# zyddnys/sd_animation_optical_flow

Hardware: AMD Instinct MI355X
Metric: frame-pairs/sec (flow+warp+mask) at 512x768 (higher is better)
Workload: dtype f32

## Files before the change

sd_animation_optical_flow_amd/csrc/conv_wino.hip:

```cpp
#include "ofx_internal.h"

#include <cmath>
#include <cstdlib>
#include <cstring>

namespace {

constexpr int kWBK = 16;
constexpr int kLDV = kWBK + 4;
constexpr int kOOB = 0x7FFFFFF0;

template <int W_, int H_, int LDH, int Y0, int X0> struct Halo {
    static constexpr int W = W_, H = H_, ldh = LDH, y_org = Y0, x_org = X0;
    static constexpr int pix = W * H;
    static constexpr int items = pix * (kWBK / 4);
    static constexpr int slots = (items + 255) / 256;
    static constexpr int floats = pix * ldh;
};
using Halo3x3 = Halo<18, 10, 24, -1, -1>;
template <bool VERT> using Halo15 = Halo<VERT ? 16 : 20, VERT ? 12 : 8, VERT ? 16 : 20, VERT ? -2 : 0, VERT ? 0 : -2>;

struct WinoK {
    const float* in0;
    const float* in1;
    const float* u;
    const float* scale;
    const float* shift;
    const float* addend;
    const float* res;
    const float* nmean;
    const float* nrstd;
    float* stats;
    float* out;
    float* aux_z;
    float* aux_rh;
    float* aux_h;
    int ld0, c0, ld1, cin, ldo, ldadd, ldh, ldres;
    int H, W, Cout, act;
    int nblk;
    int nb32;
    int tpr, tpi, mtiles;
    int bytes0, bytes1, bytesu;
    float alpha;
};

struct Patch {
    int nb, pb, y0, x0;
};

__device__ __forceinline__ Patch wino_patch(const WinoK& p) {
    const int nblk = p.mtiles * p.nblk;
    const int bid = blockIdx.x;
    const int q8 = nblk >> 3, r8 = nblk & 7;
    const int xcd = bid & 7, idx = bid >> 3;
    const int L = (xcd < r8 ? xcd * (q8 + 1) : r8 * (q8 + 1) + (xcd - r8) * q8) + idx;
    const int nb = L % p.nblk, mt = L / p.nblk;
    const int pb = mt / p.tpi;
    const int trem = mt - pb * p.tpi;
    const int py = trem / p.tpr;
    return {nb, pb, py * 8, (trem - py * p.tpr) * 16};
}

template <class ALG, bool NORM = false>
__device__ __forceinline__ void wino_slabs(const WinoK& p, const Patch& pt, float* Hs, float* Vs, int tid, int wave,
                                           f32x16 (&acc)[ALG::P][ALG::NT]) {
    typedef int v4i __attribute__((ext_vector_type(4)));
    using HALO = typename ALG::HALO;
    constexpr int P = ALG::P, NT = ALG::NT;
    const int lane = tid & 63;

    const float* in1s = p.in1 ? p.in1 : p.in0;
    const int bytes1s = p.in1 ? p.bytes1 : p.bytes0;
    int hpix[HALO::slots];
    unsigned hok = 0;
#pragma unroll
    for (int k = 0; k < HALO::slots; ++k) {
        const int i = tid + 256 * k;
        const int pix = i >> 2;
        const int hy = pix / HALO::W, hx = pix - hy * HALO::W;
        const int gy = pt.y0 + HALO::y_org + hy, gx = pt.x0 + HALO::x_org + hx;
        const bool ok = i < HALO::items && (unsigned)gy < (unsigned)p.H && (unsigned)gx < (unsigned)p.W;
        hpix[k] = ok ? (pt.pb * p.H + gy) * p.W + gx : 0;
        hok |= (ok ? 1u : 0u) << k;
    }
    const int hq = (tid & 3) * 16;
    float4 pa[HALO::slots];
    float4 pmu, prs;
    auto a_issue = [&](int cb) __attribute__((always_inline)) {
        const int c = cb * kWBK;
        const bool s0 = c < p.c0;
        const __amdgpu_buffer_rsrc_t rs = __builtin_amdgcn_make_buffer_rsrc((void*)(s0 ? p.in0 : in1s), (short)0, s0 ? p.bytes0 : bytes1s, 0x00020000);
        const int so = (s0 ? c : c - p.c0) * 4;
        const int ldb = (s0 ? p.ld0 : p.ld1) * 4;
#pragma unroll
        for (int k = 0; k < HALO::slots; ++k) {
            const int vo = ((hok >> k) & 1u) ? hpix[k] * ldb + hq : kOOB;
            v4i t = __builtin_amdgcn_raw_buffer_load_b128(rs, vo, so, 0);
            pa[k] = *reinterpret_cast<float4*>(&t);
        }
        if constexpr (NORM) {
            const long at = (long)pt.pb * p.c0 + c + (tid & 3) * 4;
            pmu = *reinterpret_cast<const float4*>(p.nmean + at);
            prs = *reinterpret_cast<const float4*>(p.nrstd + at);
        }
    };

    const __amdgpu_buffer_rsrc_t rsu = __builtin_amdgcn_make_buffer_rsrc((void*)p.u, (short)0, p.bytesu, 0x00020000);
    const int c8n = p.cin >> 3;
    const int wlane = lane * 16;
    const int pt0 = ALG::pt0(wave), blk0 = ALG::blk0(pt.nb, wave);
    float4 wr[P][NT][2];
    auto w_issue = [&](int q, int cb) __attribute__((always_inline)) {
#pragma unroll
        for (int nt = 0; nt < NT; ++nt)
#pragma unroll
            for (int ks = 0; ks < 2; ++ks) {
                const int so = (((pt0 + q) * p.nb32 + blk0 + nt) * c8n + 2 * cb + ks) * 1024;
                v4i t = __builtin_amdgcn_raw_buffer_load_b128(rsu, wlane, so, 0);
                wr[q][nt][ks] = *reinterpret_cast<float4*>(&t);
            }
    };

#pragma unroll
    for (int q = 0; q < P; ++q)
#pragma unroll
        for (int nt = 0; nt < NT; ++nt)
#pragma unroll
            for (int e = 0; e < 16; ++e) acc[q][nt][e] = 0.f;

    const ALG xf(Hs, Vs, tid, wave);
    const float* const afrag = Vs + (pt0 * 32 + (lane & 31)) * kLDV + 4 * (lane >> 5);

    const int CB = p.cin / kWBK;
    a_issue(0);
#pragma unroll
    for (int q = 0; q < P; ++q) w_issue(q, 0);
    for (int cb = 0; cb < CB; ++cb) {
        const int nx = cb + 1 < CB ? cb + 1 : cb;
#pragma unroll
        for (int k = 0; k < HALO::slots; ++k) {
            const int i = tid + 256 * k;
            if (HALO::slots * 256 > HALO::items && k == HALO::slots - 1 && i >= HALO::items) break;
            float4 v = pa[k];
            if constexpr (NORM) {
                v.x = fmaxf((v.x - pmu.x) * prs.x, 0.f);
                v.y = fmaxf((v.y - pmu.y) * prs.y, 0.f);
                v.z = fmaxf((v.z - pmu.z) * prs.z, 0.f);
                v.w = fmaxf((v.w - pmu.w) * prs.w, 0.f);
                if (!((hok >> k) & 1u)) v = make_float4(0.f, 0.f, 0.f, 0.f);
            }
            *reinterpret_cast<float4*>(&Hs[(i >> 2) * HALO::ldh + (i & 3) * 4]) = v;
        }
        __syncthreads();
        xf();
        __syncthreads();
        a_issue(nx);
        __builtin_amdgcn_sched_barrier(0);
#pragma unroll
        for (int q = 0; q < P; ++q) {
#pragma unroll
            for (int ks = 0; ks < 2; ++ks) {
                const float4 a = *reinterpret_cast<const float4*>(afrag + q * 32 * kLDV + 8 * ks);
#pragma unroll
                for (int nt = 0; nt < NT; ++nt) {
                    const float4 b = wr[q][nt][ks];
                    acc[q][nt] = __builtin_amdgcn_mfma_f32_32x32x2f32(a.x, b.x, acc[q][nt], 0, 0, 0);
                    acc[q][nt] = __builtin_amdgcn_mfma_f32_32x32x2f32(a.y, b.y, acc[q][nt], 0, 0, 0);
                    acc[q][nt] = __builtin_amdgcn_mfma_f32_32x32x2f32(a.z, b.z, acc[q][nt], 0, 0, 0);
                    acc[q][nt] = __builtin_amdgcn_mfma_f32_32x32x2f32(a.w, b.w, acc[q][nt], 0, 0, 0);
                }
            }
            w_issue(q, nx);
        }
    }
}

__device__ __forceinline__ float2 f2(float a, float b) { return make_float2(a, b); }
__device__ __forceinline__ float2 operator+(float2 a, float2 b) { return f2(a.x + b.x, a.y + b.y); }
__device__ __forceinline__ float2 operator-(float2 a, float2 b) { return f2(a.x - b.x, a.y - b.y); }
__device__ __forceinline__ float2 operator*(float s, float2 a) { return f2(s * a.x, s * a.y); }

struct Wino3x3 {
    using HALO = Halo3x3;
    static constexpr int P = 4, NT = 2;
    __device__ static int pt0(int wave) { return 4 * wave; }
    __device__ static int blk0(int nb, int) { return 2 * nb; }
    const float* src;
    float* dst;
    __device__ __forceinline__ Wino3x3(const float* Hs, float* Vs, int tid, int wave) {
        const int ttx = (tid & 63) >> 3, tcp = tid & 7;
        src = Hs + (2 * wave * HALO::W + 2 * ttx) * HALO::ldh + 2 * tcp;
        dst = Vs + (wave * 8 + ttx) * kLDV + 2 * tcp;
    }
    __device__ __forceinline__ void operator()() const {
        float2 d[4][4];
#pragma unroll
        for (int r = 0; r < 4; ++r)
#pragma unroll
            for (int c = 0; c < 4; ++c) d[r][c] = *reinterpret_cast<const float2*>(src + (r * HALO::W + c) * HALO::ldh);
        float2 t[4][4];
#pragma unroll
        for (int c = 0; c < 4; ++c) {
            t[0][c] = d[0][c] - d[2][c];
            t[1][c] = d[1][c] + d[2][c];
            t[2][c] = d[2][c] - d[1][c];
            t[3][c] = d[1][c] - d[3][c];
        }
#pragma unroll
        for (int i = 0; i < 4; ++i) {
            float2 v[4];
            v[0] = t[i][0] - t[i][2];
            v[1] = t[i][1] + t[i][2];
            v[2] = t[i][2] - t[i][1];
            v[3] = t[i][1] - t[i][3];
#pragma unroll
            for (int j = 0; j < 4; ++j) *reinterpret_cast<float2*>(dst + (i * 4 + j) * 32 * kLDV) = v[j];
        }
    }
};

template <bool VERT> struct Wino15 {
    using HALO = Halo15<VERT>;
    static constexpr int P = 8, NT = 1;
    __device__ static int pt0(int) { return 0; }
    __device__ static int blk0(int nb, int wave) { return 4 * nb + wave; }
    static constexpr int tap = (VERT ? HALO::W : 1) * HALO::ldh;
    const float* src;
    float* dst;
    __device__ static int base(int t) { return VERT ? (4 * (t >> 4)) * HALO::W + (t & 15) : (t >> 2) * HALO::W + 4 * (t & 3); }
    __device__ static int oy(int t, int i) { return VERT ? 4 * (t >> 4) + i : t >> 2; }
    __device__ static int ox(int t, int i) { return VERT ? (t & 15) : 4 * (t & 3) + i; }
    __device__ __forceinline__ Wino15(const float* Hs, float* Vs, int tid, int) {
        const int ttile = tid >> 3, tcp = tid & 7;
        src = Hs + base(ttile) * HALO::ldh + 2 * tcp;
        dst = Vs + ttile * kLDV + 2 * tcp;
    }
    __device__ __forceinline__ void operator()() const {
        float2 d[8];
#pragma unroll
        for (int j = 0; j < 8; ++j) d[j] = *reinterpret_cast<const float2*>(src + j * tap);
        float2 v[8];
        v[0] = (d[0] - d[6]) + 5.25f * (d[4] - d[2]);
        v[7] = (d[7] - d[1]) + 5.25f * (d[3] - d[5]);
        float2 te = (d[2] + d[6]) - 4.25f * d[4], to = (d[1] + d[5]) - 4.25f * d[3];
        v[1] = te + to;
        v[2] = te - to;
        te = (0.25f * d[2] + d[6]) - 1.25f * d[4];
        to = (0.5f * d[1] - 2.5f * d[3]) + 2.0f * d[5];
        v[3] = te + to;
        v[4] = te - to;
        te = (4.0f * d[2] + d[6]) - 5.0f * d[4];
        to = (2.0f * d[1] - 2.5f * d[3]) + 0.5f * d[5];
        v[5] = te + to;
        v[6] = te - to;
#pragma unroll
        for (int j = 0; j < 8; ++j) *reinterpret_cast<float2*>(dst + j * 32 * kLDV) = v[j];
    }
};

constexpr int kLDX = 32;
constexpr int kVF2 = 16 * 32 * kLDV;
constexpr int kSmem2 = Halo3x3::floats + kVF2;
constexpr int kXF = 4 * 2 * 32 * kLDX;
static_assert(kXF + 2 * 4 * 32 * 2 <= kSmem2, "exchange and statistics must fit");

template <bool NORM, bool RES, bool STATS>
__global__ __launch_bounds__(256, 2) void wino_conv_kernel(const WinoK p) {
    __shared__ __attribute__((aligned(16))) float smem[kSmem2];
    float* const Hs = smem;
    float* const Vs = smem + Halo3x3::floats;
    const int tid = threadIdx.x, lane = tid & 63;
    const int wave = __builtin_amdgcn_readfirstlane(tid >> 6);
    const Patch pt = wino_patch(p);
    f32x16 acc[4][2];
    wino_slabs<Wino3x3, NORM>(p, pt, Hs, Vs, tid, wave, acc);

    const float act_lo = p.act == OFX_ACT_RELU ? 0.0f : -3.402823466e38f;
    float* const X = smem;
    float* const Sx = smem + kXF;
    const int on = tid & 31, otx = tid >> 5;
#pragma unroll
    for (int nt = 0; nt < 2; ++nt) {
        __syncthreads();
#pragma unroll
        for (int e = 0; e < 16; ++e) {
            const int tile = (e & 3) + 8 * (e >> 2) + 4 * (lane >> 5);
            const float m0 = acc[0][nt][e], m1 = acc[1][nt][e], m2 = acc[2][nt][e], m3 = acc[3][nt][e];
            X[((wave * 2 + 0) * 32 + tile) * kLDX + (lane & 31)] = m0 + m1 + m2;
            X[((wave * 2 + 1) * 32 + tile) * kLDX + (lane & 31)] = m1 - m2 - m3;
        }
        __syncthreads();
        const int oc = pt.nb * 64 + nt * 32 + on;
        if (oc < p.Cout) {
            const float sc = (p.scale ? p.scale[oc] : 1.0f) * p.alpha;
            const float sh = p.shift ? p.shift[oc] : 0.0f;
            float st_s = 0.0f, st_q = 0.0f;
#pragma unroll
            for (int ty = 0; ty < 4; ++ty) {
                const int tile = ty * 8 + otx;
                float x[4][2];
#pragma unroll
                for (int w = 0; w < 4; ++w)
#pragma unroll
                    for (int j = 0; j < 2; ++j) x[w][j] = X[((w * 2 + j) * 32 + tile) * kLDX + on];
                float r[2][2];
                if constexpr (RES) {
#pragma unroll
                    for (int a = 0; a < 2; ++a)
#pragma unroll
                        for (int j = 0; j < 2; ++j)
                            r[a][j] = p.res[(((long)pt.pb * p.H + pt.y0 + 2 * ty + a) * p.W + pt.x0 + 2 * otx + j) * p.ldres + oc];
                }
#pragma unroll
                for (int a = 0; a < 2; ++a)
#pragma unroll
                    for (int j = 0; j < 2; ++j) {
                        const float y = a == 0 ? x[0][j] + x[1][j] + x[2][j] : x[1][j] - x[2][j] - x[3][j];
                        const long pix = ((long)pt.pb * p.H + pt.y0 + 2 * ty + a) * p.W + pt.x0 + 2 * otx + j;
                        float v = fmaxf(y * sc + sh, act_lo);
                        if constexpr (RES) v = fmaxf(v + r[a][j], 0.0f);
                        p.out[pix * p.ldo + oc] = v;
                        if constexpr (STATS) {
                            st_s += v;
                            st_q = fmaf(v, v, st_q);
                        }
                    }
            }
            if constexpr (STATS) {
                st_s += __shfl_xor(st_s, 32, 64);
                st_q += __shfl_xor(st_q, 32, 64);
                if (lane < 32) {
                    Sx[((nt * 4 + wave) * 32 + on) * 2 + 0] = st_s;
                    Sx[((nt * 4 + wave) * 32 + on) * 2 + 1] = st_q;
                }
            }
        }
    }
    if constexpr (STATS) {
        __syncthreads();
        const int nt = tid >> 5;
        const int oc = pt.nb * 64 + nt * 32 + on;
        if (tid < 64 && oc < p.Cout) {
            float s = 0.0f, q = 0.0f;
#pragma unroll
            for (int w = 0; w < 4; ++w) {
                s += Sx[((nt * 4 + w) * 32 + on) * 2 + 0];
                q += Sx[((nt * 4 + w) * 32 + on) * 2 + 1];
            }
            const long row = (long)pt.pb * p.tpi + (pt.y0 >> 3) * p.tpr + (pt.x0 >> 4);
            p.stats[(row * p.Cout + oc) * 2 + 0] = s;
            p.stats[(row * p.Cout + oc) * 2 + 1] = q;
        }
    }
}

int launch3x3(const WinoK& k, dim3 grid, dim3 block, hipStream_t s) {
    const int v = (k.nmean ? 4 : 0) | (k.res ? 2 : 0) | (k.stats ? 1 : 0);
    switch (v) {
        case 0: OFX_LAUNCH((wino_conv_kernel<false, false, false>), grid, block, s, k); break;
        case 1: OFX_LAUNCH((wino_conv_kernel<false, false, true>), grid, block, s, k); break;
        case 2: OFX_LAUNCH((wino_conv_kernel<false, true, false>), grid, block, s, k); break;
        case 4: OFX_LAUNCH((wino_conv_kernel<true, false, false>), grid, block, s, k); break;
        case 5: OFX_LAUNCH((wino_conv_kernel<true, false, true>), grid, block, s, k); break;
        case 6: OFX_LAUNCH((wino_conv_kernel<true, true, false>), grid, block, s, k); break;
        default: return OFX_EINVAL;
    }
    return ofx_launch_status();
}

template <bool VERT, int EPI>
__global__ __launch_bounds__(256, 2) void wino15_conv_kernel(const WinoK p) {
    using T = Wino15<VERT>;
    using HALO = typename T::HALO;
    __shared__ __attribute__((aligned(16))) float smem[HALO::floats + 8 * 32 * kLDV];
    float* const Hs = smem;
    float* const Vs = smem + HALO::floats;
    const int tid = threadIdx.x, lane = tid & 63;
    const int wave = __builtin_amdgcn_readfirstlane(tid >> 6);
    const Patch pt = wino_patch(p);
    f32x16 acc[8][1];
    wino_slabs<T>(p, pt, Hs, Vs, tid, wave, acc);

    const int n = pt.nb * 128 + wave * 32 + (lane & 31);
    if (n >= p.Cout) return;
    const float sc = (p.scale ? p.scale[n] : 1.0f) * p.alpha;
    const float sh = p.shift ? p.shift[n] : 0.0f;
    const float act_lo = p.act == OFX_ACT_RELU ? 0.0f : -3.402823466e38f;
    const int hd = p.Cout >> 1;
    const bool r_half = EPI == OFX_EPI_GRU_ZR && pt.nb * 128 >= hd;
#pragma unroll
    for (int eb = 0; eb < 16; eb += 4) {
        long pix[4][4];
        float y[4][4], ad[4][4], x1[4][4], x2[4][4];
#pragma unroll
        for (int u = 0; u < 4; ++u) {
            const int e = eb + u;
            const int tile = (e & 3) + 8 * (e >> 2) + 4 * (lane >> 5);
#pragma unroll
            for (int i = 0; i < 4; ++i) pix[u][i] = ((long)pt.pb * p.H + pt.y0 + T::oy(tile, i)) * p.W + pt.x0 + T::ox(tile, i);
            const float m0 = acc[0][0][e], m1 = acc[1][0][e], m2 = acc[2][0][e], m3 = acc[3][0][e];
            const float m4 = acc[4][0][e], m5 = acc[5][0][e], m6 = acc[6][0][e], m7 = acc[7][0][e];
            const float s12 = m1 + m2, d12 = m1 - m2, s34 = m3 + m4, d34 = m3 - m4, s56 = m5 + m6, d56 = m5 - m6;
            y[u][0] = m0 + s12 + s34 + s56;
            y[u][1] = d12 + 2.0f * d34 + 0.5f * d56;
            y[u][2] = s12 + 4.0f * s34 + 0.25f * s56;
            y[u][3] = d12 + 8.0f * d34 + 0.125f * d56 + m7;
        }
#pragma unroll
        for (int u = 0; u < 4; ++u)
#pragma unroll
            for (int i = 0; i < 4; ++i) {
                ad[u][i] = p.addend ? p.addend[pix[u][i] * p.ldadd + n] : 0.0f;
                x1[u][i] = EPI == OFX_EPI_GRU_ZR ? (r_half ? p.aux_h[pix[u][i] * p.ldh + n - hd] : 1.0f)
                           : EPI == OFX_EPI_GRU_Q ? p.aux_z[pix[u][i] * p.Cout + n] : 0.0f;
                x2[u][i] = EPI == OFX_EPI_GRU_Q ? p.aux_h[pix[u][i] * p.ldh + n] : 0.0f;
            }
#pragma unroll
        for (int u = 0; u < 4; ++u)
#pragma unroll
            for (int i = 0; i < 4; ++i) {
                const float v = y[u][i] * sc + sh + ad[u][i];
                if (EPI == OFX_EPI_PLAIN) {
                    p.out[pix[u][i] * p.ldo + n] = fmaxf(v, act_lo);
                } else if (EPI == OFX_EPI_GRU_ZR) {
                    const float g = ofx_sigmoid(v) * x1[u][i];
                    if (r_half) p.aux_rh[pix[u][i] * hd + n - hd] = g;
                    else p.aux_z[pix[u][i] * hd + n] = g;
                } else {
                    p.aux_h[pix[u][i] * p.ldh + n] = (1.0f - x1[u][i]) * x2[u][i] + x1[u][i] * ofx_tanh(v);
                }
            }
    }
}

template <bool VERT>
int launch15(const WinoK& k, int epi, dim3 grid, dim3 block, hipStream_t s) {
    switch (epi) {
        case OFX_EPI_PLAIN: OFX_LAUNCH((wino15_conv_kernel<VERT, OFX_EPI_PLAIN>), grid, block, s, k); break;
        case OFX_EPI_GRU_ZR: OFX_LAUNCH((wino15_conv_kernel<VERT, OFX_EPI_GRU_ZR>), grid, block, s, k); break;
        case OFX_EPI_GRU_Q: OFX_LAUNCH((wino15_conv_kernel<VERT, OFX_EPI_GRU_Q>), grid, block, s, k); break;
        default: return OFX_EINVAL;
    }
    return ofx_launch_status();
}

bool is_3x3(const ofx_conv_desc* d) { return d->KH == 3 && d->KW == 3; }
bool is_1d(int KH, int KW) { return (KH == 1 && KW == 5) || (KH == 5 && KW == 1); }
int wino_points(const ofx_conv_desc* d) { return is_3x3(d) ? 16 : 8; }
int wino_cblk(const ofx_conv_desc* d) { return is_3x3(d) ? 64 : 128; }

}

bool ofx_conv_wino_fits(const ofx_conv_desc* d) {
    const int cin = d->c0 + d->c1;
    const bool plain = d->epi == OFX_EPI_PLAIN && d->out != nullptr && d->ldo >= d->Cout && (d->act == OFX_ACT_NONE || d->act == OFX_ACT_RELU);
    bool shape_epi = false;
    if (is_3x3(d)) {
        shape_epi = d->padH == 1 && d->padW == 1 && plain && !d->addend && (!d->res || d->ldres >= d->Cout) &&
                    (!d->nmean || (d->nrstd && !d->in1 && ofx_aligned16(d->nmean) && ofx_aligned16(d->nrstd)));
    } else if (is_1d(d->KH, d->KW)) {
        shape_epi = d->padH == d->KH / 2 && d->padW == d->KW / 2 && !d->nmean && !d->res &&
                    (plain || (d->epi == OFX_EPI_GRU_ZR && (d->Cout / 2) % 128 == 0) || d->epi == OFX_EPI_GRU_Q);
    }
    return shape_epi && d->precision == OFX_PREC_FP32 && (d->nz <= 1) && d->stride == 1 && d->Hout == d->Hin && d->Wout == d->Win &&
           d->Hin % 8 == 0 && d->Win % 16 == 0 && cin % kWBK == 0 && d->c0 % kWBK == 0 &&
           d->wino_w != nullptr && ofx_aligned16(d->wino_w);
}

int ofx_conv_wino_stats_rows(const ofx_conv_desc* d) {
    return is_3x3(d) && d->act == OFX_ACT_NONE && !d->res ? (d->Hin / 8) * (d->Win / 16) : 0;
}

bool ofx_conv_wino_pays(const ofx_conv_desc* d) {
    const long patches = (long)d->B * (d->Hin / 8) * (d->Win / 16);
    return is_3x3(d) ? patches * ((d->Cout + 63) / 64) >= 1024 : patches >= 256;
}

double ofx_conv_wino_flops(const ofx_conv_desc* d) {
    return 2.0 * wino_points(d) * ((double)d->B * d->Hout * d->Wout / 4.0) * (double)(d->c0 + d->c1) * d->Cout;
}

int ofx_conv_wino_launch(const ofx_conv_desc* d, float alpha, float* stats, hipStream_t s) {
    OFX_REQUIRE(!stats || ofx_conv_wino_stats_rows(d) > 0, OFX_EINVAL);
    WinoK k;
    k.in0 = d->in0; k.in1 = d->in1; k.u = d->wino_w; k.scale = d->scale; k.shift = d->shift; k.addend = d->addend; k.out = d->out;
    k.res = d->res; k.nmean = d->nmean; k.nrstd = d->nrstd; k.stats = stats;
    k.aux_z = d->aux_z; k.aux_rh = d->aux_rh; k.aux_h = d->aux_h;
    k.ld0 = d->ld0; k.c0 = d->c0; k.ld1 = d->ld1; k.cin = d->c0 + d->c1; k.ldo = d->ldo; k.ldadd = d->ldadd; k.ldh = d->ldh;
    k.ldres = d->ldres;
    k.H = d->Hin; k.W = d->Win; k.Cout = d->Cout; k.act = d->act;
    const int cblk = wino_cblk(d);
    k.nblk = (d->Cout + cblk - 1) / cblk;
    k.nb32 = cblk / 32 * k.nblk;
    k.tpr = d->Win / 16;
    k.tpi = (d->Hin / 8) * k.tpr;
    const long mtiles = (long)d->B * k.tpi;
    const long npix = (long)d->B * d->Hin * d->Win;
    const long ext0 = ((npix - 1) * d->ld0 + d->c0) * 4, ext1 = d->in1 ? ((npix - 1) * d->ld1 + d->c1) * 4 : 0;
    const long extu = (long)wino_points(d) * k.nb32 * 32 * k.cin * 4;
    OFX_REQUIRE(ext0 < (1L << 31) - 64 && ext1 < (1L << 31) - 64 && extu < (1L << 31) - 64, OFX_EINVAL);
    OFX_REQUIRE(mtiles * k.nblk < (1L << 31) && (!is_3x3(d) || npix * d->ldo < (1L << 31)), OFX_EINVAL);
    k.mtiles = (int)mtiles;
    k.bytes0 = (int)ext0; k.bytes1 = (int)ext1; k.bytesu = (int)extu;
    k.alpha = alpha;
    const dim3 grid((unsigned)(k.mtiles * k.nblk), 1, 1), block(256, 1, 1);
    if (is_3x3(d)) return launch3x3(k, grid, block, s);
    return d->KH == 5 ? launch15<true>(k, d->epi, grid, block, s) : launch15<false>(k, d->epi, grid, block, s);
}

namespace {

template <class XF>
long wino_weight(const float* w, int Cout, int Cin, int taps, int points, int cblk, float* out, XF xf) {
    OFX_REQUIRE(Cout > 0 && Cin > 0 && Cin % kWBK == 0, OFX_EINVAL);
    const int nb32 = cblk / 32 * ((Cout + cblk - 1) / cblk);
    const long n = (long)points * nb32 * 32 * Cin;
    if (!out) return n;
    OFX_REQUIRE(w != nullptr, OFX_EINVAL);
    std::memset(out, 0, (size_t)n * sizeof(float));
    double u[16];
    for (int o = 0; o < Cout; ++o)
        for (int c = 0; c < Cin; ++c) {
            xf(w + ((size_t)o * Cin + c) * taps, u);
            for (int q = 0; q < points; ++q) {
                const long at = ((((long)q * nb32 + o / 32) * (Cin / 8) + c / 8) * 2 + (c % 8) / 4) * 128 + 4 * (o % 32) + c % 4;
                out[at] = (float)u[q];
            }
        }
    return n;
}

}

extern "C" long ofx_wino_conv_weight(const float* w, int Cout, int Cin, float* out) {
    return wino_weight(w, Cout, Cin, 9, 16, 64, out, [](const float* g, double* u) {
        static const double G[4][3] = {{1, 0, 0}, {0.5, 0.5, 0.5}, {0.5, -0.5, 0.5}, {0, 0, 1}};
        double gg[4][3];
        for (int i = 0; i < 4; ++i)
            for (int x = 0; x < 3; ++x) gg[i][x] = G[i][0] * g[x] + G[i][1] * g[3 + x] + G[i][2] * g[6 + x];
        for (int i = 0; i < 4; ++i)
            for (int j = 0; j < 4; ++j) u[4 * i + j] = gg[i][0] * G[j][0] + gg[i][1] * G[j][1] + gg[i][2] * G[j][2];
    });
}

extern "C" long ofx_wino15_conv_weight(const float* w, int Cout, int Cin, int KH, int KW, float* out) {
    OFX_REQUIRE(is_1d(KH, KW), OFX_EINVAL);
    return wino_weight(w, Cout, Cin, 5, 8, 128, out, [](const float* g, double* u) {
        static const double G[8][5] = {
            {1, 0, 0, 0, 0},
            {-2.0 / 9, -2.0 / 9, -2.0 / 9, -2.0 / 9, -2.0 / 9},
            {-2.0 / 9, 2.0 / 9, -2.0 / 9, 2.0 / 9, -2.0 / 9},
            {1.0 / 90, 1.0 / 45, 2.0 / 45, 4.0 / 45, 8.0 / 45},
            {1.0 / 90, -1.0 / 45, 2.0 / 45, -4.0 / 45, 8.0 / 45},
            {32.0 / 45, 16.0 / 45, 8.0 / 45, 4.0 / 45, 2.0 / 45},
            {32.0 / 45, -16.0 / 45, 8.0 / 45, -4.0 / 45, 2.0 / 45},
            {0, 0, 0, 0, 1},
        };
        for (int q = 0; q < 8; ++q) {
            u[q] = 0.0;
            for (int t = 0; t < 5; ++t) u[q] += G[q][t] * (double)g[t];
        }
    });
}
```

Baseline: 302.6.

## Pair two Winograd tiles per 512-thread block with phase-offset barriers

Each 512-thread workgroup now holds two independent 256-thread halves, each with its own shared-memory region and output tile. The second half starts two barrier phases behind the first, and an extra barrier sits halfway through the MFMA loop, so one half's LDS transform phase overlaps the other half's matrix-core phase. Inactive halves only spin on matching barrier counts. This doubles LDS per block and makes correctness depend on exact barrier counts matching between halves, including the epilogue. A compile-time cycle-counter probe and an env var to keep the old unpaired path are also added.

```diff
diff --git a/sd_animation_optical_flow_amd/csrc/conv_wino.hip b/sd_animation_optical_flow_amd/csrc/conv_wino.hip
--- a/sd_animation_optical_flow_amd/csrc/conv_wino.hip
+++ b/sd_animation_optical_flow_amd/csrc/conv_wino.hip
@@ -42,27 +42,67 @@
     int tpr, tpi, mtiles;
     int bytes0, bytes1, bytesu;
     float alpha;
+#ifdef OFX_WINO_PHASE_PROBE
+    unsigned long long* probe;
+    int probe_wg0, probe_wgs, probe_slabs;
+#endif
 };
 
 struct Patch {
     int nb, pb, y0, x0;
+    bool live;
 };
 
-__device__ __forceinline__ Patch wino_patch(const WinoK& p) {
-    const int nblk = p.mtiles * p.nblk;
+template <bool PAIR> constexpr int kWinoThreads = PAIR ? 512 : 256;
+
+template <bool PAIR> __device__ __forceinline__ Patch wino_patch(const WinoK& p, int half) {
+    const int items = p.mtiles * p.nblk;
+    const int nblk = PAIR ? (items + 1) >> 1 : items;
     const int bid = blockIdx.x;
     const int q8 = nblk >> 3, r8 = nblk & 7;
     const int xcd = bid & 7, idx = bid >> 3;
-    const int L = (xcd < r8 ? xcd * (q8 + 1) : r8 * (q8 + 1) + (xcd - r8) * q8) + idx;
+    int L = (xcd < r8 ? xcd * (q8 + 1) : r8 * (q8 + 1) + (xcd - r8) * q8) + idx;
+    if (PAIR) L = 2 * L + half;
+    const bool live = L < items;
+    if (!live) L = items - 1;
     const int nb = L % p.nblk, mt = L / p.nblk;
     const int pb = mt / p.tpi;
     const int trem = mt - pb * p.tpi;
     const int py = trem / p.tpr;
-    return {nb, pb, py * 8, (trem - py * p.tpr) * 16};
-}
-
-template <class ALG, bool NORM = false>
-__device__ __forceinline__ void wino_slabs(const WinoK& p, const Patch& pt, float* Hs, float* Vs, int tid, int wave,
+    return {nb, pb, py * 8, (trem - py * p.tpr) * 16, live};
+}
+
+__device__ __forceinline__ void wino_phase_barrier() {
+    __builtin_amdgcn_sched_barrier(0);
+    __builtin_amdgcn_s_barrier();
+    __builtin_amdgcn_sched_barrier(0);
+}
+
+__device__ __forceinline__ int wino_slab_barriers(int CB) { return 4 * CB + 2; }
+
+__device__ __forceinline__ void wino_idle_half(int barriers) {
+    for (int i = 0; i < barriers; ++i) __builtin_amdgcn_s_barrier();
+}
+
+#ifdef OFX_WINO_PHASE_PROBE
+__device__ __forceinline__ void wino_probe(const WinoK& p, int wave8, int slot) {
+    const int wg = (int)blockIdx.x - p.probe_wg0;
+    if (p.probe && wg >= 0 && wg < p.probe_wgs && slot < 1 + 6 * p.probe_slabs) {
+        __builtin_amdgcn_sched_barrier(0);
+        unsigned long long t = __builtin_readcyclecounter();
+        if (slot == 0)
+            t = (unsigned long long)__builtin_amdgcn_s_getreg((32 - 1) << 11 | 4) | (unsigned long long)__builtin_amdgcn_s_getreg((4 - 1) << 11 | 20) << 32;
+        if ((threadIdx.x & 63) == 0) p.probe[((long)wg * 8 + wave8) * (1 + 6 * p.probe_slabs) + slot] = t;
+        __builtin_amdgcn_sched_barrier(0);
+    }
+}
+#define WINO_PROBE(edge) wino_probe(p, 4 * half + wave, 1 + 6 * cb + (edge))
+#else
+#define WINO_PROBE(edge) ((void)0)
+#endif
+
+template <class ALG, bool NORM, bool PAIR>
+__device__ __forceinline__ void wino_slabs(const WinoK& p, const Patch& pt, float* Hs, float* Vs, int tid, int wave, int half,
                                            f32x16 (&acc)[ALG::P][ALG::NT]) {
     typedef int v4i __attribute__((ext_vector_type(4)));
     using HALO = typename ALG::HALO;
@@ -135,8 +175,13 @@
     a_issue(0);
 #pragma unroll
     for (int q = 0; q < P; ++q) w_issue(q, 0);
+    if (PAIR && half == 1) {
+        wino_phase_barrier();
+        wino_phase_barrier();
+    }
     for (int cb = 0; cb < CB; ++cb) {
         const int nx = cb + 1 < CB ? cb + 1 : cb;
+        WINO_PROBE(0);
 #pragma unroll
         for (int k = 0; k < HALO::slots; ++k) {
             const int i = tid + 256 * k;
@@ -152,12 +197,19 @@
             *reinterpret_cast<float4*>(&Hs[(i >> 2) * HALO::ldh + (i & 3) * 4]) = v;
         }
         __syncthreads();
+        WINO_PROBE(1);
         xf();
         __syncthreads();
+        WINO_PROBE(2);
         a_issue(nx);
         __builtin_amdgcn_sched_barrier(0);
 #pragma unroll
         for (int q = 0; q < P; ++q) {
+            if (q == P / 2) {
+                WINO_PROBE(3);
+                if (PAIR) wino_phase_barrier();
+                WINO_PROBE(4);
+            }
 #pragma unroll
             for (int ks = 0; ks < 2; ++ks) {
                 const float4 a = *reinterpret_cast<const float4*>(afrag + q * 32 * kLDV + 8 * ks);
@@ -172,6 +224,12 @@
             }
             w_issue(q, nx);
         }
+        WINO_PROBE(5);
+        if (PAIR) wino_phase_barrier();
+    }
+    if (PAIR && half == 0) {
+        wino_phase_barrier();
+        wino_phase_barrier();
     }
 }
 
@@ -264,16 +322,22 @@
 constexpr int kXF = 4 * 2 * 32 * kLDX;
 static_assert(kXF + 2 * 4 * 32 * 2 <= kSmem2, "exchange and statistics must fit");
 
-template <bool NORM, bool RES, bool STATS>
-__global__ __launch_bounds__(256, 2) void wino_conv_kernel(const WinoK p) {
-    __shared__ __attribute__((aligned(16))) float smem[kSmem2];
+template <bool NORM, bool RES, bool STATS, bool PAIR>
+__global__ __launch_bounds__(kWinoThreads<PAIR>, 2) void wino_conv_kernel(const WinoK p) {
+    __shared__ __attribute__((aligned(16))) float smem_all[(PAIR ? 2 : 1) * kSmem2];
+    const int tid = threadIdx.x & 255, lane = tid & 63;
+    const int wave = __builtin_amdgcn_readfirstlane(tid >> 6);
+    const int half = PAIR ? __builtin_amdgcn_readfirstlane(threadIdx.x >> 8) : 0;
+    float* const smem = smem_all + half * kSmem2;
     float* const Hs = smem;
     float* const Vs = smem + Halo3x3::floats;
-    const int tid = threadIdx.x, lane = tid & 63;
-    const int wave = __builtin_amdgcn_readfirstlane(tid >> 6);
-    const Patch pt = wino_patch(p);
+    const Patch pt = wino_patch<PAIR>(p, half);
+    if (PAIR && !pt.live) {
+        wino_idle_half(wino_slab_barriers(p.cin / kWBK) + 4 + (STATS ? 1 : 0));
+        return;
+    }
     f32x16 acc[4][2];
-    wino_slabs<Wino3x3, NORM>(p, pt, Hs, Vs, tid, wave, acc);
+    wino_slabs<Wino3x3, NORM, PAIR>(p, pt, Hs, Vs, tid, wave, half, acc);
 
     const float act_lo = p.act == OFX_ACT_RELU ? 0.0f : -3.402823466e38f;
     float* const X = smem;
@@ -354,32 +418,39 @@
     }
 }
 
+template <bool PAIR>
 int launch3x3(const WinoK& k, dim3 grid, dim3 block, hipStream_t s) {
     const int v = (k.nmean ? 4 : 0) | (k.res ? 2 : 0) | (k.stats ? 1 : 0);
     switch (v) {
-        case 0: OFX_LAUNCH((wino_conv_kernel<false, false, false>), grid, block, s, k); break;
-        case 1: OFX_LAUNCH((wino_conv_kernel<false, false, true>), grid, block, s, k); break;
-        case 2: OFX_LAUNCH((wino_conv_kernel<false, true, false>), grid, block, s, k); break;
-        case 4: OFX_LAUNCH((wino_conv_kernel<true, false, false>), grid, block, s, k); break;
-        case 5: OFX_LAUNCH((wino_conv_kernel<true, false, true>), grid, block, s, k); break;
-        case 6: OFX_LAUNCH((wino_conv_kernel<true, true, false>), grid, block, s, k); break;
+        case 0: OFX_LAUNCH((wino_conv_kernel<false, false, false, PAIR>), grid, block, s, k); break;
+        case 1: OFX_LAUNCH((wino_conv_kernel<false, false, true, PAIR>), grid, block, s, k); break;
+        case 2: OFX_LAUNCH((wino_conv_kernel<false, true, false, PAIR>), grid, block, s, k); break;
+        case 4: OFX_LAUNCH((wino_conv_kernel<true, false, false, PAIR>), grid, block, s, k); break;
+        case 5: OFX_LAUNCH((wino_conv_kernel<true, false, true, PAIR>), grid, block, s, k); break;
+        case 6: OFX_LAUNCH((wino_conv_kernel<true, true, false, PAIR>), grid, block, s, k); break;
         default: return OFX_EINVAL;
     }
     return ofx_launch_status();
 }
 
-template <bool VERT, int EPI>
-__global__ __launch_bounds__(256, 2) void wino15_conv_kernel(const WinoK p) {
+template <bool VERT, int EPI, bool PAIR>
+__global__ __launch_bounds__(kWinoThreads<PAIR>, 2) void wino15_conv_kernel(const WinoK p) {
     using T = Wino15<VERT>;
     using HALO = typename T::HALO;
-    __shared__ __attribute__((aligned(16))) float smem[HALO::floats + 8 * 32 * kLDV];
-    float* const Hs = smem;
-    float* const Vs = smem + HALO::floats;
-    const int tid = threadIdx.x, lane = tid & 63;
+    constexpr int kSmem = HALO::floats + 8 * 32 * kLDV;
+    __shared__ __attribute__((aligned(16))) float smem_all[(PAIR ? 2 : 1) * kSmem];
+    const int tid = threadIdx.x & 255, lane = tid & 63;
     const int wave = __builtin_amdgcn_readfirstlane(tid >> 6);
-    const Patch pt = wino_patch(p);
+    const int half = PAIR ? __builtin_amdgcn_readfirstlane(threadIdx.x >> 8) : 0;
+    float* const Hs = smem_all + half * kSmem;
+    float* const Vs = Hs + HALO::floats;
+    const Patch pt = wino_patch<PAIR>(p, half);
+    if (PAIR && !pt.live) {
+        wino_idle_half(wino_slab_barriers(p.cin / kWBK));
+        return;
+    }
     f32x16 acc[8][1];
-    wino_slabs<T>(p, pt, Hs, Vs, tid, wave, acc);
+    wino_slabs<T, false, PAIR>(p, pt, Hs, Vs, tid, wave, half, acc);
 
     const int n = pt.nb * 128 + wave * 32 + (lane & 31);
     if (n >= p.Cout) return;
@@ -433,12 +504,12 @@
     }
 }
 
-template <bool VERT>
+template <bool VERT, bool PAIR>
 int launch15(const WinoK& k, int epi, dim3 grid, dim3 block, hipStream_t s) {
     switch (epi) {
-        case OFX_EPI_PLAIN: OFX_LAUNCH((wino15_conv_kernel<VERT, OFX_EPI_PLAIN>), grid, block, s, k); break;
-        case OFX_EPI_GRU_ZR: OFX_LAUNCH((wino15_conv_kernel<VERT, OFX_EPI_GRU_ZR>), grid, block, s, k); break;
-        case OFX_EPI_GRU_Q: OFX_LAUNCH((wino15_conv_kernel<VERT, OFX_EPI_GRU_Q>), grid, block, s, k); break;
+        case OFX_EPI_PLAIN: OFX_LAUNCH((wino15_conv_kernel<VERT, OFX_EPI_PLAIN, PAIR>), grid, block, s, k); break;
+        case OFX_EPI_GRU_ZR: OFX_LAUNCH((wino15_conv_kernel<VERT, OFX_EPI_GRU_ZR, PAIR>), grid, block, s, k); break;
+        case OFX_EPI_GRU_Q: OFX_LAUNCH((wino15_conv_kernel<VERT, OFX_EPI_GRU_Q, PAIR>), grid, block, s, k); break;
         default: return OFX_EINVAL;
     }
     return ofx_launch_status();
@@ -448,6 +519,10 @@
 bool is_1d(int KH, int KW) { return (KH == 1 && KW == 5) || (KH == 5 && KW == 1); }
 int wino_points(const ofx_conv_desc* d) { return is_3x3(d) ? 16 : 8; }
 int wino_cblk(const ofx_conv_desc* d) { return is_3x3(d) ? 64 : 128; }
+#ifdef OFX_WINO_PHASE_PROBE
+unsigned long long* g_probe = nullptr;
+int g_probe_wg0 = 0, g_probe_wgs = 0, g_probe_slabs = 0;
+#endif
 
 }
 
@@ -503,10 +578,26 @@
     k.mtiles = (int)mtiles;
     k.bytes0 = (int)ext0; k.bytes1 = (int)ext1; k.bytesu = (int)extu;
     k.alpha = alpha;
-    const dim3 grid((unsigned)(k.mtiles * k.nblk), 1, 1), block(256, 1, 1);
-    if (is_3x3(d)) return launch3x3(k, grid, block, s);
-    return d->KH == 5 ? launch15<true>(k, d->epi, grid, block, s) : launch15<false>(k, d->epi, grid, block, s);
-}
+#ifdef OFX_WINO_PHASE_PROBE
+    k.probe = g_probe; k.probe_wg0 = g_probe_wg0; k.probe_wgs = g_probe_wgs; k.probe_slabs = g_probe_slabs;
+#endif
+    static const bool unpaired = getenv("OFX_CONV_WINO_UNPAIRED") != nullptr;
+    const long items = mtiles * k.nblk;
+    if (unpaired) {
+        const dim3 grid((unsigned)items, 1, 1), block(kWinoThreads<false>, 1, 1);
+        if (is_3x3(d)) return launch3x3<false>(k, grid, block, s);
+        return d->KH == 5 ? launch15<true, false>(k, d->epi, grid, block, s) : launch15<false, false>(k, d->epi, grid, block, s);
+    }
+    const dim3 grid((unsigned)((items + 1) / 2), 1, 1), block(kWinoThreads<true>, 1, 1);
+    if (is_3x3(d)) return launch3x3<true>(k, grid, block, s);
+    return d->KH == 5 ? launch15<true, true>(k, d->epi, grid, block, s) : launch15<false, true>(k, d->epi, grid, block, s);
+}
+
+#ifdef OFX_WINO_PHASE_PROBE
+extern "C" void ofx_wino_phase_probe(void* buf, int wg0, int wgs, int slabs) {
+    g_probe = (unsigned long long*)buf; g_probe_wg0 = wg0; g_probe_wgs = wgs; g_probe_slabs = slabs;
+}
+#endif
 
 namespace {
 
```

Measured after the change: 296.7 (median of 2 runs). -1.9%, worse.
